# alvinliu0/HumanGaussian

Measured on AMD Instinct MI355X. Metric: rasterize fwd+bwd Gaussians/sec @1024^2, 100k pts, higher is better.
Workload: dtype f32

## Files before the change

humangaussian_amd/csrc/api.hip:

```cpp
#include "hgs_common.h"
#include <stdio.h>
#include <stdlib.h>
#include <string.h>
#include <algorithm>
#include <atomic>
#include <mutex>

#ifdef HGS_TIMELINE
__device__ unsigned long long hgs_tl[HGS_TL_KERNELS][HGS_TL_SLOTS][4];
#endif
#include "preprocess.hip"
#include "binning.hip"
#include "render_fwd.hip"
#include "knn.hip"
#include "mesh.hip"
#include "fields.hip"
#include "bookkeeping.hip"
#include "optim.hip"
#include "lbs.hip"
#include "pose.hip"
#include "step_images.hip"
#include "surface.hip"

extern "C" __global__ void hgs_k_render_bwd(View, Layout, const hgs_status*, const SortRec*, const float*,
// ... 4 lines not shown

namespace {

#ifdef HGS_KNOBS
inline int hgs_knob(const char* name, int dflt) { const char* e = getenv(name); return (e && atoi(e) > 0) ? atoi(e) : dflt; }
#else
inline int hgs_knob(const char*, int dflt) { return dflt; }
#endif

#define HGS_CHUNK_ROWS_MIN_VIEWS 3
#ifndef HGS_PRE_BWD_VPAR_MIN_VIEWS
#define HGS_PRE_BWD_VPAR_MIN_VIEWS 2
#endif
constexpr size_t ALIGN = 256;
struct Carver {
  size_t off = 0;
  size_t take(size_t bytes) { const size_t o = off; off = hgs_align_up(off + bytes, ALIGN); return o; }
};
struct ScanShape { unsigned blocks; size_t bsum_bytes; };
inline ScanShape scan_shape(size_t n, size_t elem) {
  const size_t nb = (n + HGS_SCAN_BLOCK - 1) / HGS_SCAN_BLOCK;
  return {(unsigned)nb, (nb + 1) * elem};
}
constexpr size_t HGS_LDS_BINS_MAX = 16384;
#define HGS_BIN_WGS_PER_VIEW_MAX 512
#define HGS_BIN_WGS_TOTAL_MAX 1024
constexpr int HGS_MAX_BIN_WGS_PER_VIEW = HGS_BIN_WGS_PER_VIEW_MAX;
constexpr int HGS_BIN_WGS_TOTAL = HGS_BIN_WGS_TOTAL_MAX;

struct GeomCarve {
  size_t geom, tile_n, tile_start, tile_order, tile_rec, cell_info, items_part, fwd_cells,
      hist, tile_gbase, tile_count, chunk_sums, chunk_base, ctr, status, total;
};

inline int grid_dim(int pixels) { return (pixels + HGS_TILE - 1) / HGS_TILE; }

inline void bin_shape(int B, int P, int& nblk, int& cpw, int& nwg) {
  nblk = (P + HGS_BLOCK - 1) / HGS_BLOCK;
  int want = HGS_BIN_WGS_TOTAL / (B > 0 ? B : 1);
  if (want > HGS_MAX_BIN_WGS_PER_VIEW) want = HGS_MAX_BIN_WGS_PER_VIEW;
  if (want < 1) want = 1;
  cpw = (nblk + want - 1) / want;
  if (cpw < 1) cpw = 1;
  nwg = (nblk + cpw - 1) / cpw;
}

GeomCarve carve_geom(int B, int P, int H, int W) {
  const size_t T = (size_t)grid_dim(W) * grid_dim(H);
  const size_t TT = T * (size_t)B;
  int nblk, cpw, nwg;
  bin_shape(B, P, nblk, cpw, nwg);
  const bool lds = T <= HGS_LDS_BINS_MAX;
  GeomCarve c;
  Carver cv;
  c.geom = cv.take((size_t)B * P * sizeof(GeomRec));
  c.tile_n = cv.take(TT * 4);
  c.tile_start = cv.take(TT * 4);
  c.tile_order = cv.take(TT * 4);
  c.tile_rec = cv.take(TT * 16);
  c.cell_info = cv.take(TT * 16 * sizeof(CellInfo));
  const size_t dcap = hgs_die_cells((int)TT);
  c.items_part = cv.take(HGS_NXCD * 2 * dcap * sizeof(uint4));
  c.fwd_cells = cv.take((size_t)HGS_NXCD * HGS_NFC * dcap * 4);
  c.hist = cv.take(lds ? (size_t)B * nwg * T * 4 : 0);
  c.tile_gbase = cv.take(lds ? (size_t)HGS_ROW_GROUPS * TT * 4 : 0);
  c.tile_count = cv.take(lds ? 0 : TT * 4);
  c.chunk_sums = cv.take((size_t)B * nblk * 4);
  c.chunk_base = cv.take((size_t)B * nblk * 4);
  c.ctr = cv.take(sizeof(Counters));
  c.status = cv.take(sizeof(hgs_status));
  c.total = cv.off;
  return c;
}

// ... 25 lines not shown
  L.tile_start = reinterpret_cast<uint32_t*>(gp + g.tile_start);
  L.tile_order = reinterpret_cast<uint32_t*>(gp + g.tile_order);
  L.tile_rec = reinterpret_cast<uint4*>(gp + g.tile_rec);
  L.cell_info = reinterpret_cast<CellInfo*>(gp + g.cell_info);
  L.items_part = reinterpret_cast<uint4*>(gp + g.items_part);
  L.fwd_cells = reinterpret_cast<uint32_t*>(gp + g.fwd_cells);
  L.hist = reinterpret_cast<uint32_t*>(gp + g.hist);
  L.tile_gbase = reinterpret_cast<uint32_t*>(gp + g.tile_gbase);
  L.tile_count = reinterpret_cast<uint32_t*>(gp + g.tile_count);
  L.chunk_sums = reinterpret_cast<uint32_t*>(gp + g.chunk_sums);
  L.chunk_base = reinterpret_cast<uint32_t*>(gp + g.chunk_base);
  L.ctr = reinterpret_cast<Counters*>(gp + g.ctr);
  L.keys = bp ? reinterpret_cast<unsigned long long*>(bp + b.keys) : nullptr;
  L.recs = bp ? reinterpret_cast<SortRec*>(bp + b.recs) : nullptr;
  L.cell_list = bp ? reinterpret_cast<uint2*>(bp + b.cell_list) : nullptr;
  L.entpair = bp ? reinterpret_cast<uint2*>(bp + b.entpair) : nullptr;
  L.cstate = bp ? reinterpret_cast<float*>(bp + b.cstate) : nullptr;
  L.items_full = bp ? reinterpret_cast<uint4*>(bp + b.items_full) : nullptr;
  L.full_cap = (uint32_t)((size_t)(cap > 0 ? cap : 0) * HGS_PAIRS_PER_ENTRY / HGS_SEGLEN + 1);
  L.n_contrib = static_cast<uint32_t*>(img);
  return L;
}

View make_view(const hgs_settings* s, int B, int P, int M, int64_t cap, int max_tile_hint = 0, int act = 0) {
  View v;
  v.act = act;
  v.pairchunks = B >= HGS_CHUNK_ROWS_MIN_VIEWS ? 1 : 0;
  for (int b = 0; b < HGS_MAX_VIEWS; ++b) {
    const hgs_settings& sb = s[b < B ? b : 0];
    Cam& c = v.cam[b];
    c.viewmatrix = sb.viewmatrix;
    c.projmatrix = sb.projmatrix;
    c.campos = sb.campos;
    c.bg = sb.bg;
    c.tanfovx = sb.tanfovx;
    c.tanfovy = sb.tanfovy;
    c.focal_x = (float)sb.image_width / (2.0f * sb.tanfovx);
    c.focal_y = (float)sb.image_height / (2.0f * sb.tanfovy);
  }
  v.scale_modifier = s->scale_modifier;
  v.W = s->image_width;
  v.H = s->image_height;
  v.grid_x = grid_dim(v.W);
  v.grid_y = grid_dim(v.H);
  v.T = v.grid_x * v.grid_y;
  v.B = B;
  v.TT = B * v.T;
  v.P = P;
  v.M = M;
  v.D = s->sh_degree;
  v.lds_bins = (size_t)v.T <= HGS_LDS_BINS_MAX ? 1 : 0;
  bin_shape(B, P, v.nblk, v.cpw, v.nwg);
  if (!v.lds_bins) { v.cpw = 1; v.nwg = v.nblk; }
  v.entry_capacity = (uint32_t)(cap < 0 ? 0 : (cap > 0xffffffffll ? 0xffffffffll : cap));
  v.max_tile_hint = max_tile_hint;
  return v;
}

inline int hip_rc(hipError_t e) { return e == hipSuccess ? HGS_OK : -(1000 + (int)e); }

inline hipError_t box_init(void* hdr, size_t hdr_bytes, uint32_t* bmin, hipStream_t stream) {
  const hipError_t e = hipMemsetAsync(hdr, 0, hdr_bytes, stream);
  return e != hipSuccess ? e : hipMemsetAsync(bmin, 0xff, 3 * sizeof(uint32_t), stream);
}

#define HGS_LAUNCH_CHECK()                       \
  do {                                           \
    hipError_t e__ = hipGetLastError();          \
    if (e__ != hipSuccess) return hip_rc(e__);   \
  } while (0)

#define HGS_STAGE(k)                                                              \
  do {                                                                            \
    if (stage_events && stage_events[k]) {                                        \
      hipError_t e__ = hipEventRecord(static_cast<hipEvent_t>(stage_events[k]), stream); \
// ... 240 lines not shown

int hgs_forward_batch_act(const hgs_settings* s, int32_t B, int32_t P, int32_t M, const float* means3D,
                          const float* shs, const float* colors_precomp, const float* opacities,
                          const float* scales, const float* rotations, const float* cov3D_precomp,
                          float* out_color, float* out_depth, float* out_alpha, int32_t* radii,
                          void* geom, void* bin, int64_t entry_capacity, void* img,
                          int32_t store_bwd_state, int32_t max_tile_entries_hint, hgs_status* status_host,
                          int32_t status_host_mapped, void* status_event, void* const* stage_events,
                          int32_t activation_flags, void* stream_) {
  return hgs_forward_batch_act_leaf(s, B, P, M, means3D, shs, colors_precomp, opacities, scales, rotations, cov3D_precomp,
                                    out_color, out_depth, out_alpha, radii, geom, bin, entry_capacity, img, store_bwd_state,
                                    max_tile_entries_hint, status_host, status_host_mapped, status_event, stage_events,
                                    activation_flags, nullptr, stream_);
}

int hgs_forward_batch_act_leaf(const hgs_settings* s, int32_t B, int32_t P, int32_t M, const float* means3D,
                               const float* shs, const float* colors_precomp, const float* opacities,
                               const float* scales, const float* rotations, const float* cov3D_precomp,
                               float* out_color, float* out_depth, float* out_alpha, int32_t* radii,
                               void* geom, void* bin, int64_t entry_capacity, void* img,
                               int32_t store_bwd_state, int32_t max_tile_entries_hint, hgs_status* status_host,
                               int32_t status_host_mapped, void* status_event, void* const* stage_events,
                               int32_t activation_flags, float* means2D_leaf, void* stream_) {
  if (activation_flags & ~(7 | HGS_GRAD_SCALE_TRUE_DERIVATIVE | HGS_ANTIALIAS)) return HGS_EINVAL;
  if (!batch_ok(s, B) || P < 0 || !out_color || !out_depth || !out_alpha || !geom || !img ||
      entry_capacity < 0)
    return HGS_EINVAL;
  if (P > 0) {
    if (!means3D || !opacities || !radii) return HGS_EINVAL;
    if ((shs != nullptr) == (colors_precomp != nullptr)) return HGS_ESHAPE;
    const bool has_sr = scales != nullptr && rotations != nullptr;
    if ((scales != nullptr) != (rotations != nullptr)) return HGS_ESHAPE;
    if (has_sr == (cov3D_precomp != nullptr)) return HGS_ESHAPE;
    if (shs && M < (s->sh_degree + 1) * (s->sh_degree + 1)) return HGS_ESHAPE;
    if (entry_capacity > 0 && !bin) return HGS_EINVAL;
    if ((int64_t)B * P >= (1ll << 31) || P >= (1 << 28)) return HGS_EINVAL;
  }
  if (entry_capacity > HGS_MAX_ENTRY_CAPACITY) return HGS_EINVAL;
  hipStream_t stream = static_cast<hipStream_t>(stream_);
  DeviceState* const ds = device_state(stream);
  const int ncu = cu_count(ds);
  const bool aa = (activation_flags & HGS_ANTIALIAS) != 0;
  const View v = make_view(s, B, P, M, entry_capacity, max_tile_entries_hint > 0 ? max_tile_entries_hint : 0,
                           activation_flags & 7);
  const Layout L = make_layout(geom, bin, img, B, P, v.H, v.W, entry_capacity);
  hgs_status* status_dev =
      reinterpret_cast<hgs_status*>(static_cast<char*>(geom) + carve_geom(B, P, v.H, v.W).status);

  HGS_STAGE(0);
  hipError_t e = hipSuccess;
  if (v.nblk == 0) {
    e = hipMemsetAsync(L.ctr, 0, sizeof(Counters), stream);
    if (e != hipSuccess) return hip_rc(e);
  }
  const size_t lds_bytes = (size_t)v.T * 4;
  if (!v.lds_bins) {
    e = hipMemsetAsync(L.tile_count, 0, (size_t)v.TT * 4, stream);
    if (e != hipSuccess) return hip_rc(e);
  }
  if (v.nblk > 0) {
    if (v.lds_bins)
      hipLaunchKernelGGL(aa ? hgs_k_preprocess_fwd_aa : hgs_k_preprocess_fwd, dim3(v.B * v.nwg), dim3(HGS_BLOCK), lds_bytes,
                         stream, v, L, means3D, shs, colors_precomp, opacities, scales, rotations,
                         cov3D_precomp, radii, means2D_leaf);
    else
      hipLaunchKernelGGL(aa ? hgs_k_preprocess_fwd_ga_aa : hgs_k_preprocess_fwd_ga, dim3(v.B * v.nblk), dim3(HGS_BLOCK), 0,
                         stream, v, L, means3D, shs, colors_precomp, opacities, scales, rotations,
                         cov3D_precomp, radii, means2D_leaf);
    HGS_LAUNCH_CHECK();
  }
  HGS_STAGE(1);
  const unsigned bpv = (unsigned)((v.T + HGS_TILES_PER_WG - 1) / HGS_TILES_PER_WG);
  hipLaunchKernelGGL(hgs_k_tiles, dim3(bpv * (unsigned)v.B), dim3(64 * HGS_ROW_GROUPS), 0, stream, v, L);
  HGS_LAUNCH_CHECK();
  HGS_STAGE(2);
  const unsigned order_wgs = (unsigned)((v.TT + HGS_BLOCK - 1) / HGS_BLOCK);
  hgs_status* status_mapped = status_host_mapped ? status_host : nullptr;
  const unsigned nbin = entry_capacity > 0 ? (unsigned)(v.B * (v.lds_bins ? v.nwg : v.nblk)) : 0u;
  if (v.lds_bins && nbin)
    hipLaunchKernelGGL(hgs_k_fill, dim3(nbin + order_wgs), dim3(HGS_BLOCK), lds_bytes, stream, v, L, status_dev,
                       status_mapped, (int)nbin);
  else
    hipLaunchKernelGGL(hgs_k_fill_ga, dim3(nbin + order_wgs), dim3(HGS_BLOCK), 0, stream, v, L, status_dev,
                       status_mapped, (int)nbin);
  HGS_LAUNCH_CHECK();
  if (status_host && !status_host_mapped) {
    e = hipMemcpyAsync(status_host, status_dev, sizeof(hgs_status), hipMemcpyDeviceToHost, stream);
    if (e != hipSuccess) return hip_rc(e);
  }
  if (status_event) {
    e = hipEventRecord(static_cast<hipEvent_t>(status_event), stream);
    if (e != hipSuccess) return hip_rc(e);
  }
  if (entry_capacity > 0) {
    HGS_STAGE(3);
    auto class_grid = [&](int64_t lo) {
      const int64_t g = entry_capacity / lo + 1;
      return (unsigned)(g < v.TT ? g : v.TT);
    };
    const int hint = v.max_tile_hint;
    const bool need_huge = hint <= 0 || hint > 16384, need_large = hint <= 0 || hint > HGS_SORT_LDS_MAX;
    const bool expect_long = hint <= 0 || hint > HGS_SORT_LDS_MAX + HGS_SORT_LDS_MAX / 2 + 64;
// ... 909 lines not shown
```

humangaussian_amd/csrc/binning.hip:

```cpp
#include "hgs_common.h"

extern "C" __global__ void __launch_bounds__(64 * HGS_ROW_GROUPS)
hgs_k_tiles(View v, Layout L) {
  __shared__ uint32_t gt[HGS_ROW_GROUPS][HGS_TILES_PER_WG];
  __shared__ uint32_t start_s[HGS_TILES_PER_WG];
  __shared__ uint32_t cls_s[HGS_NCLS];
  const int tid = threadIdx.x, tl = tid & 63;
  const int rg = __builtin_amdgcn_readfirstlane(tid >> 6);
  const int bpv = (v.T + HGS_TILES_PER_WG - 1) / HGS_TILES_PER_WG;
  const int b = (int)blockIdx.x / bpv;
  const int t = ((int)blockIdx.x % bpv) * HGS_TILES_PER_WG + tl;
  const bool valid = t < v.T;
  const size_t g = (size_t)b * v.T + t;
  if (tid < HGS_NCLS) cls_s[tid] = 0;
  uint32_t run = 0;
  if (v.lds_bins) {
    const int rpg = (v.nwg + HGS_ROW_GROUPS - 1) / HGS_ROW_GROUPS;
    const int r0 = rg * rpg, r1 = min(v.nwg, r0 + rpg);
    if (valid) {
      uint32_t* col = L.hist + (size_t)b * v.nwg * v.T + t;
      constexpr int BR = 16;
      for (int r = r0; r < r1; r += BR) {
        uint32_t c[BR];
#pragma unroll
// ... 77 lines not shown
      const uint32_t* sw = reinterpret_cast<const uint32_t*>(&st);
      for (int k = 0; k < 7; ++k) hs[k] = sw[k];
      __threadfence_system();
      hs[7] = 1u;
      __threadfence_system();
    }
  }
  if (tid >= 128 && tid < 192) {
    const int nchunk = v.B * v.nblk;
    const int per_wg = (nchunk + nblks - 1) / nblks;
    const int c_begin = blk * per_wg, c_end = min(nchunk, c_begin + per_wg);
    for (int c0 = c_begin; c0 < c_end; c0 += 64) {
      const int c = c0 + lane;
      const uint32_t sum = (c < c_end) ? L.chunk_sums[c] : 0u;
      const uint32_t inc = hgs_wave_incl_scan(sum);
      uint32_t base = 0;
      if (lane == 63 && inc) base = atomicAdd(&L.ctr->entry_alloc, inc);
      base = (uint32_t)__builtin_amdgcn_readlane((int)base, 63);
      if (c < c_end) L.chunk_base[c] = base + inc - sum;
    }
  }
  __syncthreads();
  const int g = blk * HGS_BLOCK + tid;
  const bool valid = g < v.TT;
  const uint32_t n = valid ? L.tile_n[g] : 0u;
  const int c = (valid && n) ? 32 - __clz(n) : 0;
  int leader_of = 0;
  uint32_t rank = 0, cnt = 0;
  unsigned long long todo = __ballot(valid);
  while (todo) {
    const int leader = (int)__builtin_ctzll(todo);
    const int cl = __builtin_amdgcn_readlane(c, leader);
    const unsigned long long same = __ballot(valid && c == cl);
    if (valid && c == cl) {
      leader_of = leader;
      rank = __builtin_amdgcn_mbcnt_hi((uint32_t)(same >> 32), __builtin_amdgcn_mbcnt_lo((uint32_t)same, 0u));
      cnt = (uint32_t)__popcll(same);
    }
    todo &= ~same;
  }
  uint32_t base = 0;
  if (valid && lane == leader_of) base = atomicAdd(&L.ctr->cls_cur[c].v, cnt);
  base = (uint32_t)__shfl((int)base, leader_of, 64);
  const uint32_t pos = cls_base[c] + base + rank;
  if (!valid) return;
  L.tile_order[pos] = (uint32_t)g;
  L.tile_rec[pos] = make_uint4((uint32_t)g, n, L.tile_start[g], 0u);
}

extern "C" __global__ void __launch_bounds__(HGS_BLOCK)
hgs_k_fill(View v, Layout L, hgs_status* __restrict__ status, hgs_status* __restrict__ status_host, int nbin) {
  extern __shared__ __attribute__((aligned(16))) uint32_t lds_cur[];
  if ((int)blockIdx.x >= nbin) {
    place_tiles(v, L, (int)blockIdx.x - nbin, (int)gridDim.x - nbin, status, status_host);
    return;
  }
  if (overflow_from_counters(v, L)) return;
  const int b = (int)blockIdx.x / v.nwg, lw = (int)blockIdx.x % v.nwg;
  const uint32_t* __restrict__ base_row = L.hist + (size_t)blockIdx.x * v.T;
  const int rpg = (v.nwg + HGS_ROW_GROUPS - 1) / HGS_ROW_GROUPS;
  const uint32_t* __restrict__ grp_row = L.tile_gbase + (size_t)(lw / rpg) * v.TT + (size_t)b * v.T;
  for (int t = threadIdx.x; t < v.T; t += HGS_BLOCK) lds_cur[t] = grp_row[t] + base_row[t];
  __syncthreads();
  const GeomRec* __restrict__ geom = L.geom + (size_t)b * v.P;
  for (int c = 0; c < v.cpw; ++c) {
    const int chunk = lw * v.cpw + c;
    if (chunk >= v.nblk) break;
    const int i = chunk * HGS_BLOCK + threadIdx.x;
    if (i >= v.P) continue;
    const uint4 q2 = reinterpret_cast<const uint4*>(&geom[i])[2];
    const uint32_t depth_bits = q2.y, lo = q2.z, hi = q2.w;
    const int minx = lo & 0xffffu, miny = lo >> 16, maxx = hi & 0xffffu, maxy = hi >> 16;
    const unsigned long long key_hi = (unsigned long long)depth_bits << 32;
    for (int ty = miny; ty < maxy; ++ty)
      for (int tx = minx; tx < maxx; ++tx) {
        const uint32_t slot = atomicAdd(&lds_cur[ty * v.grid_x + tx], 1u);
        L.keys[slot] = key_hi | (uint32_t)i;
      }
  }
}

extern "C" __global__ void __launch_bounds__(HGS_BLOCK)
hgs_k_fill_ga(View v, Layout L, hgs_status* __restrict__ status, hgs_status* __restrict__ status_host, int nbin) {
  if ((int)blockIdx.x >= nbin) {
    place_tiles(v, L, (int)blockIdx.x - nbin, (int)gridDim.x - nbin, status, status_host);
    return;
  }
  if (overflow_from_counters(v, L)) return;
  const int b = (int)blockIdx.x / v.nblk, chunk = (int)blockIdx.x % v.nblk;
  const int i = chunk * HGS_BLOCK + threadIdx.x;
  if (i >= v.P) return;
  const uint4 q2 = reinterpret_cast<const uint4*>(&L.geom[(size_t)b * v.P + i])[2];
  const uint32_t depth_bits = q2.y, lo = q2.z, hi = q2.w;
  const int minx = lo & 0xffffu, miny = lo >> 16, maxx = hi & 0xffffu, maxy = hi >> 16;
  const unsigned long long key_hi = (unsigned long long)depth_bits << 32;
  for (int ty = miny; ty < maxy; ++ty)
    for (int tx = minx; tx < maxx; ++tx) {
      const size_t g = (size_t)b * v.T + ty * v.grid_x + tx;
      const uint32_t slot = L.tile_start[g] + atomicAdd(&L.tile_count[g], 1u);
      L.keys[slot] = key_hi | (uint32_t)i;
    }
}
// ... 966 lines not shown
```

humangaussian_amd/csrc/hgs_common.h:

```cpp
#pragma once
#include <hip/hip_runtime.h>
#include <stdint.h>

#include "../../include/hgs_rast.h"
#include "cellmask.h"
#include "entryrec.h"

#define HGS_TILE 16
#define HGS_TILE_PIX 256
#define HGS_BLOCK 256
#define HGS_ROW_GROUPS 16
#define HGS_TILES_PER_WG 64
#define HGS_RB 16
#define HGS_ROW_F4 (HGS_RB * HGS_REC_F4 + 1)
#define HGS_BWD_BLOCK_WAVES 12
#define HGS_SEGLEN 128
#define HGS_NEAR_Z 0.2f
#define HGS_ALPHA_MIN (1.0f / 255.0f)
#define HGS_ALPHA_MAX 0.99f
#define HGS_T_EPS 0.0001f
#define HGS_CSTATE_FLOATS (6 * 16)
#define HGS_ROW_FLOATS 12
#define HGS_GROW_F4 (HGS_ROW_FLOATS / 4)
#define HGS_PROW_FLOATS 10
// ... 69 lines not shown
  float* cstate;
  uint32_t full_cap;
  uint4* items_full;
  uint32_t* n_contrib;
};

__host__ __device__ __forceinline__ size_t hgs_die_cells(int TT) { return (size_t)16 * (size_t)((TT + HGS_NXCD - 1) / HGS_NXCD); }

struct Cam {
  const float* viewmatrix;
  const float* projmatrix;
  const float* campos;
  const float* bg;
  float tanfovx, tanfovy, focal_x, focal_y;
};

struct View {
  Cam cam[HGS_MAX_VIEWS];
  float scale_modifier;
  int32_t W, H, grid_x, grid_y, T;
  int32_t B, TT;
  int32_t P, M, D, nblk;
  int32_t cpw, nwg, lds_bins;
  uint32_t entry_capacity;
  int32_t max_tile_hint;
  int32_t act;
  int32_t pairchunks;
};

static inline size_t hgs_align_up(size_t v, size_t a) { return (v + a - 1) / a * a; }

__device__ __forceinline__ int hgs_cell_of(int w, int j) { return (((w >> 1) << 1) + (j >> 1)) * 4 + ((w & 1) << 1) + (j & 1); }
#define HGS_FWD_THREADS 256

__device__ __forceinline__ bool hgs_eval_alpha(float dx, float dy, float qa, float qb,
                                               float qc, float op, float& G, float& alpha,
                                               float& m2, float& m3) {
  m2 = __builtin_fmaf(qa, dx, qb * dy);
  m3 = qc * dy;
  const float p2 = __builtin_fmaf(dx, m2, m3 * dy);
  G = __builtin_amdgcn_exp2f(p2);
  const float og = op * G;
  alpha = fminf(HGS_ALPHA_MAX, og);
  return (p2 <= 0.0f) && (og >= HGS_ALPHA_MIN);
}

// ... 86 lines not shown
```

humangaussian_amd/csrc/preprocess.hip:

```cpp
#include "hgs_common.h"

namespace {

__device__ __constant__ const float SH_C0 = 0.28209479177387814f;
__device__ __constant__ const float SH_C1 = 0.4886025119029199f;
__device__ __constant__ const float SH_C2[5] = {1.0925484305920792f, -1.0925484305920792f,
                                                0.31539156525252005f, -1.0925484305920792f,
                                                0.5462742152960396f};
__device__ __constant__ const float SH_C3[7] = {-0.5900435899266435f, 2.890611442640554f,
                                                -0.4570457994644658f, 0.3731763325901154f,
                                                -0.4570457994644658f, 1.445305721320277f,
                                                -0.5900435899266435f};

struct Cov3 { float c0, c1, c2, c3, c4, c5; };

struct RotScale {
  float R00, R01, R02, R10, R11, R12, R20, R21, R22;
  float sx, sy, sz;
};

__device__ __forceinline__ float act_opacity(float raw, int act) {
  return (act & HGS_ACT_OPACITY_SIGMOID) ? 1.0f / (1.0f + expf(-raw)) : raw;
}
__device__ __forceinline__ void act_scale(const float* __restrict__ scales, int i, int act, float& s0, float& s1, float& s2) {
// ... 277 lines not shown
      col[ch] = col[ch] + 0.5f;
      if (col[ch] < 0.0f) { cl |= (1u << ch); col[ch] = 0.0f; }
    }
    rec.r = col[0]; rec.g = col[1]; rec.b = col[2];
    rec.clamped = cl;
  }
  return (uint32_t)tight_area;
}

__device__ __forceinline__ void store_geom(GeomRec* dstp, const GeomRec& rec) {
  uint4* dst = reinterpret_cast<uint4*>(dstp);
  const uint4* src = reinterpret_cast<const uint4*>(&rec);
  dst[0] = src[0]; dst[1] = src[1]; dst[2] = src[2]; dst[3] = src[3];
}

}

__device__ __forceinline__ uint32_t chunk_prefix(uint32_t tt, uint32_t* wtot, uint32_t* chunk_sum) {
  uint32_t total;
  const uint32_t ex = hgs_block_excl_scan<HGS_BLOCK>(tt, wtot, total);
  if (threadIdx.x == 0) *chunk_sum = total;
  return ex;
}

__device__ __forceinline__ void zero_counters(const Layout& L) {
  if (blockIdx.x == 0)
    for (uint32_t i = threadIdx.x; i < sizeof(Counters) / 4; i += blockDim.x) reinterpret_cast<uint32_t*>(L.ctr)[i] = 0u;
}

template <bool AA>
__device__ __forceinline__ void preprocess_fwd_body(
    const View& v, const Layout& L, const float* __restrict__ means3D, const float* __restrict__ shs,
    const float* __restrict__ colors_precomp, const float* __restrict__ opacities, const float* __restrict__ scales,
    const float* __restrict__ rotations, const float* __restrict__ cov3D_precomp, int32_t* __restrict__ radii,
    float* __restrict__ zero_leaf) {
  extern __shared__ __attribute__((aligned(16))) uint32_t lds_hist[];
  __shared__ uint32_t wtot[HGS_BLOCK / 64];
  zero_counters(L);
  const int b = (int)blockIdx.x / v.nwg, lw = (int)blockIdx.x % v.nwg;
  const Cam cam = v.cam[b];
  for (int t = threadIdx.x; t < v.T; t += HGS_BLOCK) lds_hist[t] = 0u;
  __syncthreads();
  const int gxm = v.grid_x;
  for (int c = 0; c < v.cpw; ++c) {
    const int chunk = lw * v.cpw + c;
    if (chunk >= v.nblk) break;
    const int i = chunk * HGS_BLOCK + threadIdx.x;
    uint32_t tt = 0;
    if (i < v.P) {
      GeomRec rec;
      tt = preprocess_one<AA>(v, cam, i, means3D, shs, colors_precomp, opacities, scales, rotations,
                              cov3D_precomp, rec);
      radii[(size_t)b * v.P + i] = rec.radius;
      if (zero_leaf) {
        float* z = zero_leaf + ((size_t)b * v.P + i) * 3;
        z[0] = 0.0f; z[1] = 0.0f; z[2] = 0.0f;
      }
      store_geom(&L.geom[(size_t)b * v.P + i], rec);
      if (tt) {
        const int minx = rec.rect_lo & 0xffffu, miny = rec.rect_lo >> 16;
        const int maxx = rec.rect_hi & 0xffffu, maxy = rec.rect_hi >> 16;
        for (int ty = miny; ty < maxy; ++ty)
          for (int tx = minx; tx < maxx; ++tx) atomicAdd(&lds_hist[ty * gxm + tx], 1u);
      }
    }
    const uint32_t off = chunk_prefix(tt, wtot, &L.chunk_sums[(size_t)b * v.nblk + chunk]);
    if (i < v.P && tt) L.geom[(size_t)b * v.P + i].offset = off;
  }
  __syncthreads();
  uint32_t* row = L.hist + (size_t)blockIdx.x * v.T;
  for (int t = threadIdx.x; t < v.T; t += HGS_BLOCK) row[t] = lds_hist[t];
}

template <bool AA>
__device__ __forceinline__ void preprocess_fwd_ga_body(
    const View& v, const Layout& L, const float* __restrict__ means3D, const float* __restrict__ shs,
    const float* __restrict__ colors_precomp, const float* __restrict__ opacities, const float* __restrict__ scales,
    const float* __restrict__ rotations, const float* __restrict__ cov3D_precomp, int32_t* __restrict__ radii,
    float* __restrict__ zero_leaf) {
  __shared__ uint32_t wtot[HGS_BLOCK / 64];
  zero_counters(L);
  const int b = (int)blockIdx.x / v.nblk, chunk = (int)blockIdx.x % v.nblk;
  const Cam cam = v.cam[b];
  const int i = chunk * HGS_BLOCK + threadIdx.x;
  uint32_t tt = 0;
  if (i < v.P) {
    GeomRec rec;
    tt = preprocess_one<AA>(v, cam, i, means3D, shs, colors_precomp, opacities, scales, rotations,
                            cov3D_precomp, rec);
    radii[(size_t)b * v.P + i] = rec.radius;
    if (zero_leaf) {
      float* z = zero_leaf + ((size_t)b * v.P + i) * 3;
      z[0] = 0.0f; z[1] = 0.0f; z[2] = 0.0f;
    }
    store_geom(&L.geom[(size_t)b * v.P + i], rec);
    if (tt) {
      const int minx = rec.rect_lo & 0xffffu, miny = rec.rect_lo >> 16;
      const int maxx = rec.rect_hi & 0xffffu, maxy = rec.rect_hi >> 16;
      uint32_t* cnt = L.tile_count + (size_t)b * v.T;
      for (int ty = miny; ty < maxy; ++ty)
        for (int tx = minx; tx < maxx; ++tx) atomicAdd(&cnt[ty * v.grid_x + tx], 1u);
    }
  }
  const uint32_t off = chunk_prefix(tt, wtot, &L.chunk_sums[blockIdx.x]);
  if (i < v.P && tt) L.geom[(size_t)b * v.P + i].offset = off;
}

#define HGS_PRE_FWD_KERNEL(NAME, BODY, AA)                                                                       \
  extern "C" __global__ void __launch_bounds__(HGS_BLOCK) NAME(                                                  \
      View v, Layout L, const float* __restrict__ means3D, const float* __restrict__ shs,                        \
      const float* __restrict__ colors_precomp, const float* __restrict__ opacities,                             \
      const float* __restrict__ scales, const float* __restrict__ rotations,                                     \
      const float* __restrict__ cov3D_precomp, int32_t* __restrict__ radii, float* __restrict__ zero_leaf) {     \
    BODY<AA>(v, L, means3D, shs, colors_precomp, opacities, scales, rotations, cov3D_precomp, radii, zero_leaf);   \
  }
HGS_PRE_FWD_KERNEL(hgs_k_preprocess_fwd, preprocess_fwd_body, false)
HGS_PRE_FWD_KERNEL(hgs_k_preprocess_fwd_ga, preprocess_fwd_ga_body, false)
HGS_PRE_FWD_KERNEL(hgs_k_preprocess_fwd_aa, preprocess_fwd_body, true)
HGS_PRE_FWD_KERNEL(hgs_k_preprocess_fwd_ga_aa, preprocess_fwd_ga_body, true)

namespace {

template <int DEG, int MODE, int AA>
__device__ __forceinline__ void preprocess_bwd_body(
    const View& v, const Layout& L, const hgs_status* __restrict__ status,
    const float* __restrict__ grad_rows, const float* __restrict__ means3D,
    const float* __restrict__ shs, const float* __restrict__ colors_precomp,
    const float* __restrict__ opacities_raw,
    const float* __restrict__ scales, const float* __restrict__ rotations,
    const float* __restrict__ cov3D_precomp, float* __restrict__ dL_dmeans3D,
    float* __restrict__ dL_dmeans2D, float* __restrict__ dL_dshs, float* __restrict__ dL_dcolors,
    float* __restrict__ dL_dopac, float* __restrict__ dL_dscales, float* __restrict__ dL_drots,
    float* __restrict__ dL_dcov3D, float* __restrict__ pack, int pack_F) {
  constexpr int NC = (DEG + 1) * (DEG + 1);
  constexpr bool SINGLE = MODE != 0;
  constexpr bool VPAR = MODE == 2;
  constexpr int NV = 23 + 3 * NC;
  extern __shared__ float red[];
  int i = blockIdx.x * HGS_BLOCK + threadIdx.x, bview = 0, il = threadIdx.x;
  if (VPAR) {
    il = (int)threadIdx.x & 63;
    bview = __builtin_amdgcn_readfirstlane((int)threadIdx.x >> 6);
// ... 520 lines not shown
```

humangaussian_amd/csrc/torch_binding.cpp:

```cpp
#include <torch/extension.h>
#include <c10/hip/HIPFunctions.h>
#include <c10/hip/HIPStream.h>
#include <hip/hip_runtime_api.h>

#include <algorithm>
#include <atomic>
#include <chrono>
#include <thread>
#include <map>
#include <tuple>
#include <mutex>
#include <utility>
#include <stdexcept>
#include <string>
#include <vector>

#include "../../include/hgs_rast.h"

namespace {

using torch::Tensor;
using torch::autograd::AutogradContext;
using torch::autograd::variable_list;

// ... 244 lines not shown
      const int slot = st.ring_pos;
      st.ring_pos = (st.ring_pos + 1) % RING;
      st.ring_issued += 1;
      plan->slot = &st.ring[slot];
      plan->slot_issue = st.ring_issued;
      volatile uint32_t* ready = &st.ring[slot].reserved[2];
      *ready = 0u;
      std::atomic_thread_fence(std::memory_order_seq_cst);
      const auto th1 = std::chrono::steady_clock::now();
      if (attempt == 0) st.host_ns[0] += std::chrono::duration_cast<std::chrono::nanoseconds>(th1 - th0).count();
      const int rc = hgs_forward_batch_act_leaf(plan->settings.s.data(), (int32_t)B, (int32_t)P, M, fptr(m3), fptr(sh_), fptr(cp_),
                                                fptr(op_), fptr(sc_), fptr(ro_), fptr(cv_), fptr_mut(color), fptr_mut(depth),
                                                fptr_mut(alpha), P > 0 ? radii.data_ptr<int32_t>() : nullptr, plan->geom,
                                                plan->bin, cap, plan->img, want_grad ? 1 : 0, hint, &st.ring[slot], 1,
                                                nullptr, g_stage_fwd.empty() ? nullptr : g_stage_fwd.data(),
                                                (int32_t)act, leaf_ptr, stream);
      check_rc(rc, "hgs_forward_batch");
      const auto th2 = std::chrono::steady_clock::now();
      st.host_ns[1] += std::chrono::duration_cast<std::chrono::nanoseconds>(th2 - th1).count();
      if (debug) hip_ok(hipStreamSynchronize(stream), "device error in the rasterizer forward (debug=True)");
      if (attempt == 0 && want_grad) {
        plan->B = (int32_t)B; plan->P = (int32_t)P; plan->M = M;
        plan->batched = batched;
        plan->act = (int32_t)act;
        plan->has_sh = has_sh; plan->has_cp = has_cp; plan->has_sr = has_sc; plan->has_cv = has_cv;
        plan->opac_sizes = opacities.sizes().vec();
        variable_list saved = {m3, op_, radii, color, depth, alpha};
        for (const Tensor* t : {&sh_, &cp_, &sc_, &ro_, &cv_})
          if (t->defined()) saved.push_back(*t);
        ctx->save_for_backward(saved);
        plan->alloc_grads(plan->pre_grads, dev);
        plan->pre_stream = (void*)stream;
      }
      const auto tw = std::chrono::steady_clock::now();
      st.host_ns[2] += std::chrono::duration_cast<std::chrono::nanoseconds>(tw - th2).count();
      for (uint64_t spins = 0; *ready == 0u; ++spins) {
        if ((spins & 0x3ff) == 0x3ff) {
          if (std::chrono::steady_clock::now() - tw > std::chrono::seconds(2)) {
            hip_ok(hipStreamSynchronize(stream), "rasterizer forward");
            if (*ready == 0u) throw std::runtime_error("libhgs_rast: the forward finished without publishing its status");
            break;
          }
          std::this_thread::yield();
        }
      }
      std::atomic_thread_fence(std::memory_order_seq_cst);
      const int64_t waited = std::chrono::duration_cast<std::chrono::nanoseconds>(std::chrono::steady_clock::now() - tw).count();
// ... 1135 lines not shown
```

humangaussian_amd/rasterizer.py:

```python
from __future__ import annotations

from typing import NamedTuple, Optional

import torch
from torch import nn

from . import _lib


class GaussianRasterizationSettings(NamedTuple):
    image_height: int
    image_width: int
    tanfovx: float
    tanfovy: float
    bg: torch.Tensor
    scale_modifier: float
    viewmatrix: torch.Tensor
    projmatrix: torch.Tensor
    sh_degree: int
    campos: torch.Tensor
    prefiltered: bool
    debug: bool


# ... 23 lines not shown

def rasterize_gaussians(means3D, means2D, sh, colors_precomp, opacities, scales, rotations,
                        cov3Ds_precomp, raster_settings, zero_means2D: bool = False,
                        antialiasing: Optional[bool] = None):
    want_grad = torch.is_grad_enabled() and (
        means3D.requires_grad or means2D.requires_grad or opacities.requires_grad
        or (sh is not None and sh.requires_grad)
        or (colors_precomp is not None and colors_precomp.requires_grad)
        or (scales is not None and scales.requires_grad)
        or (rotations is not None and rotations.requires_grad)
        or (cov3Ds_precomp is not None and cov3Ds_precomp.requires_grad))
    rs = raster_settings
    aa = _settings_antialiasing(rs) if antialiasing is None else bool(antialiasing)
    color, radii, depth, alpha = _lib.load_binding().rasterize(
        means3D, means2D, sh, colors_precomp, opacities, scales, rotations, cov3Ds_precomp,
        rs.bg, rs.viewmatrix, rs.projmatrix, rs.campos, int(rs.image_height), int(rs.image_width),
        float(rs.tanfovx), float(rs.tanfovy), float(rs.scale_modifier), int(rs.sh_degree),
        bool(rs.prefiltered), bool(rs.debug), want_grad, bool(zero_means2D), ANTIALIAS if aa else 0)
    return color, radii, depth, alpha


ACT_OPACITY_SIGMOID, ACT_SCALE_EXP, ACT_ROTATION_NORMALIZE = 1, 2, 4
ANTIALIAS = 16
ZERO_MEANS2D = 1 << 16
GRAD_SCALE_TRUE_DERIVATIVE = 8


def rasterize_gaussians_batch(means3D, means2D, sh, colors_precomp, opacities, scales, rotations,
                              cov3Ds_precomp, raster_settings_list, activation_flags: int = 0,
                              antialiasing: Optional[bool] = None):
    rsl = list(raster_settings_list)
    if not rsl:
        raise ValueError("rasterize_gaussians_batch needs at least one view")
    r0 = rsl[0]
    for rs in rsl[1:]:
        if (int(rs.image_height), int(rs.image_width), int(rs.sh_degree), float(rs.scale_modifier)) != \
                (int(r0.image_height), int(r0.image_width), int(r0.sh_degree), float(r0.scale_modifier)):
            raise ValueError("all views of a batch must share image size, sh_degree and scale_modifier")
        if _settings_antialiasing(rs) != _settings_antialiasing(r0):
            raise ValueError("all views of a batch must agree in antialiasing")
    if antialiasing is None:
        antialiasing = bool(int(activation_flags) & ANTIALIAS) or _settings_antialiasing(r0)
    activation_flags = (int(activation_flags) & ~ANTIALIAS) | (ANTIALIAS if antialiasing else 0)
    B = len(rsl)
    dev = means3D.device
    if B == 1:
# ... 71 lines not shown
```

include/hgs_rast.h:

```cpp
#ifndef HGS_RAST_H
#define HGS_RAST_H

#include <stddef.h>
#include <stdint.h>

#ifdef __cplusplus
extern "C" {
#endif

#define HGS_MAX_VIEWS 16
#define HGS_MAX_ENTRY_CAPACITY (1ll << 27)

#define HGS_OK 0
#define HGS_EINVAL (-1)
#define HGS_ESHAPE (-2)

typedef struct hgs_settings {
  int32_t image_height;
  int32_t image_width;
  float tanfovx;
  float tanfovy;
  const float* bg;
  float scale_modifier;
  const float* viewmatrix;
// ... 43 lines not shown
                      int32_t store_bwd_state, int32_t max_tile_entries_hint,
                      hgs_status* status_host, int32_t status_host_mapped, void* status_event,
                      void* const* stage_events, void* stream);

int hgs_backward_batch(const hgs_settings* views, int32_t B, int32_t P, int32_t M,
                       const float* means3D, const float* shs, const float* colors_precomp,
                       const float* opacities, const float* scales, const float* rotations,
                       const float* cov3D_precomp, const int32_t* radii,
                       const float* out_color, const float* out_depth, const float* out_alpha,
                       const float* dL_dout_color, const float* dL_dout_depth,
                       const float* dL_dout_alpha,
                       const void* geom, const void* bin, const void* img,
                       const hgs_status* status, int64_t entry_capacity, void* bwd_scratch,
                       float* dL_dmeans3D, float* dL_dmeans2D, float* dL_dshs,
                       float* dL_dcolors_precomp, float* dL_dopacities, float* dL_dscales,
                       float* dL_drotations, float* dL_dcov3D_precomp,
                       void* const* stage_events, void* stream);

#define HGS_ACT_OPACITY_SIGMOID 1
#define HGS_ACT_SCALE_EXP 2
#define HGS_ACT_ROTATION_NORMALIZE 4
#define HGS_GRAD_SCALE_TRUE_DERIVATIVE 8
#define HGS_ANTIALIAS 16
int hgs_forward_batch_act(const hgs_settings* views, int32_t B, int32_t P, int32_t M,
                          const float* means3D, const float* shs, const float* colors_precomp,
                          const float* opacities, const float* scales, const float* rotations,
                          const float* cov3D_precomp,
                          float* out_color, float* out_depth, float* out_alpha, int32_t* radii,
                          void* geom, void* bin, int64_t entry_capacity, void* img,
                          int32_t store_bwd_state, int32_t max_tile_entries_hint,
                          hgs_status* status_host, int32_t status_host_mapped, void* status_event,
                          void* const* stage_events, int32_t activation_flags, void* stream);
int hgs_forward_batch_act_leaf(const hgs_settings* views, int32_t B, int32_t P, int32_t M,
                               const float* means3D, const float* shs, const float* colors_precomp,
                               const float* opacities, const float* scales, const float* rotations,
                               const float* cov3D_precomp,
                               float* out_color, float* out_depth, float* out_alpha, int32_t* radii,
                               void* geom, void* bin, int64_t entry_capacity, void* img,
                               int32_t store_bwd_state, int32_t max_tile_entries_hint,
                               hgs_status* status_host, int32_t status_host_mapped, void* status_event,
                               void* const* stage_events, int32_t activation_flags, float* means2D_leaf, void* stream);
int hgs_backward_batch_act(const hgs_settings* views, int32_t B, int32_t P, int32_t M,
                           const float* means3D, const float* shs, const float* colors_precomp,
                           const float* opacities, const float* scales, const float* rotations,
                           const float* cov3D_precomp, const int32_t* radii,
                           const float* out_color, const float* out_depth, const float* out_alpha,
// ... 268 lines not shown
```

Before: 658.4 million.

## Add wide 2-chunk workgroups for single-view preprocess and binning fill

For single-view batches whose chunk count exceeds the CU count, preprocess and fill now launch workgroups of twice the block size, each processing two point chunks at once. This halves the number of per-workgroup tile histogram rows that must be zeroed, written, scanned and read back in fill. It also keeps per-chunk prefix sums correct through a new wave-grouped scan. The cost is fewer, larger workgroups and a per-workgroup LDS histogram shared by more threads, which can increase atomic contention. New flags let callers force narrow or wide mode.

```diff
diff --git a/humangaussian_amd/csrc/api.hip b/humangaussian_amd/csrc/api.hip
--- a/humangaussian_amd/csrc/api.hip
+++ b/humangaussian_amd/csrc/api.hip
@@ -50,6 +50,7 @@
   const size_t nb = (n + HGS_SCAN_BLOCK - 1) / HGS_SCAN_BLOCK;
   return {(unsigned)nb, (nb + 1) * elem};
 }
+#define HGS_BIN_BITS (HGS_BIN_NARROW | HGS_BIN_WIDE)
 constexpr size_t HGS_LDS_BINS_MAX = 16384;
 #define HGS_BIN_WGS_PER_VIEW_MAX 512
 #define HGS_BIN_WGS_TOTAL_MAX 1024
@@ -63,21 +64,29 @@
 
 inline int grid_dim(int pixels) { return (pixels + HGS_TILE - 1) / HGS_TILE; }
 
-inline void bin_shape(int B, int P, int& nblk, int& cpw, int& nwg) {
+inline void bin_shape(int B, int P, bool wide, int& nblk, int& cpw, int& nwg) {
   nblk = (P + HGS_BLOCK - 1) / HGS_BLOCK;
   int want = HGS_BIN_WGS_TOTAL / (B > 0 ? B : 1);
   if (want > HGS_MAX_BIN_WGS_PER_VIEW) want = HGS_MAX_BIN_WGS_PER_VIEW;
   if (want < 1) want = 1;
   cpw = (nblk + want - 1) / want;
   if (cpw < 1) cpw = 1;
+  if (wide) cpw = (cpw + 1) & ~1;
   nwg = (nblk + cpw - 1) / cpw;
+}
+
+inline bool bin_wide(int flags, int B, int P, int ncu) {
+  if (B != 1 || (flags & HGS_BIN_NARROW)) return false;
+  if (flags & HGS_BIN_WIDE) return true;
+  const int nblk = (P + HGS_BLOCK - 1) / HGS_BLOCK;
+  return nblk > ncu && nblk <= HGS_MAX_BIN_WGS_PER_VIEW;
 }
 
 GeomCarve carve_geom(int B, int P, int H, int W) {
   const size_t T = (size_t)grid_dim(W) * grid_dim(H);
   const size_t TT = T * (size_t)B;
   int nblk, cpw, nwg;
-  bin_shape(B, P, nblk, cpw, nwg);
+  bin_shape(B, P, false, nblk, cpw, nwg);
   const bool lds = T <= HGS_LDS_BINS_MAX;
   GeomCarve c;
   Carver cv;
@@ -149,7 +158,7 @@
   return L;
 }
 
-View make_view(const hgs_settings* s, int B, int P, int M, int64_t cap, int max_tile_hint = 0, int act = 0) {
+View make_view(const hgs_settings* s, int B, int P, int M, int64_t cap, int max_tile_hint = 0, int act = 0, bool wide = false) {
   View v;
   v.act = act;
   v.pairchunks = B >= HGS_CHUNK_ROWS_MIN_VIEWS ? 1 : 0;
@@ -177,7 +186,8 @@
   v.M = M;
   v.D = s->sh_degree;
   v.lds_bins = (size_t)v.T <= HGS_LDS_BINS_MAX ? 1 : 0;
-  bin_shape(B, P, v.nblk, v.cpw, v.nwg);
+  v.wide = (wide && v.lds_bins && B == 1) ? 1 : 0;
+  bin_shape(B, P, v.wide != 0, v.nblk, v.cpw, v.nwg);
   if (!v.lds_bins) { v.cpw = 1; v.nwg = v.nblk; }
   v.entry_capacity = (uint32_t)(cap < 0 ? 0 : (cap > 0xffffffffll ? 0xffffffffll : cap));
   v.max_tile_hint = max_tile_hint;
@@ -464,7 +474,8 @@
                                int32_t store_bwd_state, int32_t max_tile_entries_hint, hgs_status* status_host,
                                int32_t status_host_mapped, void* status_event, void* const* stage_events,
                                int32_t activation_flags, float* means2D_leaf, void* stream_) {
-  if (activation_flags & ~(7 | HGS_GRAD_SCALE_TRUE_DERIVATIVE | HGS_ANTIALIAS)) return HGS_EINVAL;
+  if (activation_flags & ~(7 | HGS_GRAD_SCALE_TRUE_DERIVATIVE | HGS_ANTIALIAS | HGS_BIN_BITS)) return HGS_EINVAL;
+  if ((activation_flags & HGS_BIN_BITS) == HGS_BIN_BITS) return HGS_EINVAL;
   if (!batch_ok(s, B) || P < 0 || !out_color || !out_depth || !out_alpha || !geom || !img ||
       entry_capacity < 0)
     return HGS_EINVAL;
@@ -484,7 +495,7 @@
   const int ncu = cu_count(ds);
   const bool aa = (activation_flags & HGS_ANTIALIAS) != 0;
   const View v = make_view(s, B, P, M, entry_capacity, max_tile_entries_hint > 0 ? max_tile_entries_hint : 0,
-                           activation_flags & 7);
+                           activation_flags & 7, bin_wide(activation_flags, B, P, ncu));
   const Layout L = make_layout(geom, bin, img, B, P, v.H, v.W, entry_capacity);
   hgs_status* status_dev =
       reinterpret_cast<hgs_status*>(static_cast<char*>(geom) + carve_geom(B, P, v.H, v.W).status);
@@ -501,7 +512,11 @@
     if (e != hipSuccess) return hip_rc(e);
   }
   if (v.nblk > 0) {
-    if (v.lds_bins)
+    if (v.wide)
+      hipLaunchKernelGGL(aa ? hgs_k_preprocess_fwd_w_aa : hgs_k_preprocess_fwd_w, dim3(v.nwg), dim3(2 * HGS_BLOCK), lds_bytes,
+                         stream, v, L, means3D, shs, colors_precomp, opacities, scales, rotations,
+                         cov3D_precomp, radii, means2D_leaf);
+    else if (v.lds_bins)
       hipLaunchKernelGGL(aa ? hgs_k_preprocess_fwd_aa : hgs_k_preprocess_fwd, dim3(v.B * v.nwg), dim3(HGS_BLOCK), lds_bytes,
                          stream, v, L, means3D, shs, colors_precomp, opacities, scales, rotations,
                          cov3D_precomp, radii, means2D_leaf);
@@ -519,7 +534,10 @@
   const unsigned order_wgs = (unsigned)((v.TT + HGS_BLOCK - 1) / HGS_BLOCK);
   hgs_status* status_mapped = status_host_mapped ? status_host : nullptr;
   const unsigned nbin = entry_capacity > 0 ? (unsigned)(v.B * (v.lds_bins ? v.nwg : v.nblk)) : 0u;
-  if (v.lds_bins && nbin)
+  if (v.wide && nbin)
+    hipLaunchKernelGGL(hgs_k_fill_w, dim3(nbin + order_wgs), dim3(2 * HGS_BLOCK), lds_bytes, stream, v, L, status_dev,
+                       status_mapped, (int)nbin);
+  else if (v.lds_bins && nbin)
     hipLaunchKernelGGL(hgs_k_fill, dim3(nbin + order_wgs), dim3(HGS_BLOCK), lds_bytes, stream, v, L, status_dev,
                        status_mapped, (int)nbin);
   else
diff --git a/humangaussian_amd/csrc/binning.hip b/humangaussian_amd/csrc/binning.hip
--- a/humangaussian_amd/csrc/binning.hip
+++ b/humangaussian_amd/csrc/binning.hip
@@ -123,7 +123,7 @@
   }
   __syncthreads();
   const int g = blk * HGS_BLOCK + tid;
-  const bool valid = g < v.TT;
+  const bool valid = g < v.TT && tid < HGS_BLOCK;
   const uint32_t n = valid ? L.tile_n[g] : 0u;
   const int c = (valid && n) ? 32 - __clz(n) : 0;
   int leader_of = 0;
@@ -149,8 +149,9 @@
   L.tile_rec[pos] = make_uint4((uint32_t)g, n, L.tile_start[g], 0u);
 }
 
-extern "C" __global__ void __launch_bounds__(HGS_BLOCK)
-hgs_k_fill(View v, Layout L, hgs_status* __restrict__ status, hgs_status* __restrict__ status_host, int nbin) {
+template <int NCH>
+__device__ __forceinline__ void fill_body(const View& v, const Layout& L, hgs_status* __restrict__ status,
+                                          hgs_status* __restrict__ status_host, int nbin) {
   extern __shared__ __attribute__((aligned(16))) uint32_t lds_cur[];
   if ((int)blockIdx.x >= nbin) {
     place_tiles(v, L, (int)blockIdx.x - nbin, (int)gridDim.x - nbin, status, status_host);
@@ -161,13 +162,14 @@
   const uint32_t* __restrict__ base_row = L.hist + (size_t)blockIdx.x * v.T;
   const int rpg = (v.nwg + HGS_ROW_GROUPS - 1) / HGS_ROW_GROUPS;
   const uint32_t* __restrict__ grp_row = L.tile_gbase + (size_t)(lw / rpg) * v.TT + (size_t)b * v.T;
-  for (int t = threadIdx.x; t < v.T; t += HGS_BLOCK) lds_cur[t] = grp_row[t] + base_row[t];
+  for (int t = threadIdx.x; t < v.T; t += NCH * HGS_BLOCK) lds_cur[t] = grp_row[t] + base_row[t];
   __syncthreads();
   const GeomRec* __restrict__ geom = L.geom + (size_t)b * v.P;
-  for (int c = 0; c < v.cpw; ++c) {
+  const int half = NCH == 1 ? 0 : (int)threadIdx.x / HGS_BLOCK, tl = (int)threadIdx.x % HGS_BLOCK;
+  for (int c = half; c < v.cpw; c += NCH) {
     const int chunk = lw * v.cpw + c;
     if (chunk >= v.nblk) break;
-    const int i = chunk * HGS_BLOCK + threadIdx.x;
+    const int i = chunk * HGS_BLOCK + tl;
     if (i >= v.P) continue;
     const uint4 q2 = reinterpret_cast<const uint4*>(&geom[i])[2];
     const uint32_t depth_bits = q2.y, lo = q2.z, hi = q2.w;
@@ -179,6 +181,14 @@
         L.keys[slot] = key_hi | (uint32_t)i;
       }
   }
+}
+extern "C" __global__ void __launch_bounds__(HGS_BLOCK)
+hgs_k_fill(View v, Layout L, hgs_status* __restrict__ status, hgs_status* __restrict__ status_host, int nbin) {
+  fill_body<1>(v, L, status, status_host, nbin);
+}
+extern "C" __global__ void __launch_bounds__(2 * HGS_BLOCK)
+hgs_k_fill_w(View v, Layout L, hgs_status* __restrict__ status, hgs_status* __restrict__ status_host, int nbin) {
+  fill_body<2>(v, L, status, status_host, nbin);
 }
 
 extern "C" __global__ void __launch_bounds__(HGS_BLOCK)
diff --git a/humangaussian_amd/csrc/hgs_common.h b/humangaussian_amd/csrc/hgs_common.h
--- a/humangaussian_amd/csrc/hgs_common.h
+++ b/humangaussian_amd/csrc/hgs_common.h
@@ -115,6 +115,7 @@
   int32_t B, TT;
   int32_t P, M, D, nblk;
   int32_t cpw, nwg, lds_bins;
+  int32_t wide;
   uint32_t entry_capacity;
   int32_t max_tile_hint;
   int32_t act;
diff --git a/humangaussian_amd/csrc/preprocess.hip b/humangaussian_amd/csrc/preprocess.hip
--- a/humangaussian_amd/csrc/preprocess.hip
+++ b/humangaussian_amd/csrc/preprocess.hip
@@ -323,32 +323,50 @@
   if (threadIdx.x == 0) *chunk_sum = total;
   return ex;
 }
+__device__ __forceinline__ uint32_t chunk_prefix_wide(uint32_t tt, uint32_t* wtot, uint32_t* chunk_sum) {
+  const int lane = threadIdx.x & 63, w = threadIdx.x >> 6, w0 = w & ~3;
+  const uint32_t incl = hgs_wave_incl_scan(tt);
+  __syncthreads();
+  if (lane == 63) wtot[w] = incl;
+  __syncthreads();
+  uint32_t base = 0, tot = 0;
+#pragma unroll
+  for (int k = 0; k < HGS_BLOCK / 64; ++k) {
+    const uint32_t t = wtot[w0 + k];
+    if (w0 + k < w) base += t;
+    tot += t;
+  }
+  if ((threadIdx.x & (HGS_BLOCK - 1)) == 0 && chunk_sum) *chunk_sum = tot;
+  return base + incl - tt;
+}
 
 __device__ __forceinline__ void zero_counters(const Layout& L) {
   if (blockIdx.x == 0)
     for (uint32_t i = threadIdx.x; i < sizeof(Counters) / 4; i += blockDim.x) reinterpret_cast<uint32_t*>(L.ctr)[i] = 0u;
 }
 
-template <bool AA>
+template <bool AA, int NCH>
 __device__ __forceinline__ void preprocess_fwd_body(
     const View& v, const Layout& L, const float* __restrict__ means3D, const float* __restrict__ shs,
     const float* __restrict__ colors_precomp, const float* __restrict__ opacities, const float* __restrict__ scales,
     const float* __restrict__ rotations, const float* __restrict__ cov3D_precomp, int32_t* __restrict__ radii,
     float* __restrict__ zero_leaf) {
   extern __shared__ __attribute__((aligned(16))) uint32_t lds_hist[];
-  __shared__ uint32_t wtot[HGS_BLOCK / 64];
+  __shared__ uint32_t wtot[NCH * HGS_BLOCK / 64];
   zero_counters(L);
   const int b = (int)blockIdx.x / v.nwg, lw = (int)blockIdx.x % v.nwg;
   const Cam cam = v.cam[b];
-  for (int t = threadIdx.x; t < v.T; t += HGS_BLOCK) lds_hist[t] = 0u;
+  for (int t = threadIdx.x; t < v.T; t += NCH * HGS_BLOCK) lds_hist[t] = 0u;
   __syncthreads();
   const int gxm = v.grid_x;
-  for (int c = 0; c < v.cpw; ++c) {
-    const int chunk = lw * v.cpw + c;
-    if (chunk >= v.nblk) break;
-    const int i = chunk * HGS_BLOCK + threadIdx.x;
+  const int half = NCH == 1 ? 0 : (int)threadIdx.x / HGS_BLOCK, tl = (int)threadIdx.x % HGS_BLOCK;
+  for (int c = 0; c < v.cpw; c += NCH) {
+    if (lw * v.cpw + c >= v.nblk) break;
+    const int chunk = lw * v.cpw + c + half;
+    const bool has = NCH == 1 || chunk < v.nblk;
+    const int i = chunk * HGS_BLOCK + tl;
     uint32_t tt = 0;
-    if (i < v.P) {
+    if (has && i < v.P) {
       GeomRec rec;
       tt = preprocess_one<AA>(v, cam, i, means3D, shs, colors_precomp, opacities, scales, rotations,
                               cov3D_precomp, rec);
@@ -365,15 +383,16 @@
           for (int tx = minx; tx < maxx; ++tx) atomicAdd(&lds_hist[ty * gxm + tx], 1u);
       }
     }
-    const uint32_t off = chunk_prefix(tt, wtot, &L.chunk_sums[(size_t)b * v.nblk + chunk]);
-    if (i < v.P && tt) L.geom[(size_t)b * v.P + i].offset = off;
+    uint32_t* const chunk_sum = &L.chunk_sums[(size_t)b * v.nblk + chunk];
+    const uint32_t off = NCH == 1 ? chunk_prefix(tt, wtot, chunk_sum) : chunk_prefix_wide(tt, wtot, has ? chunk_sum : nullptr);
+    if (has && i < v.P && tt) L.geom[(size_t)b * v.P + i].offset = off;
   }
   __syncthreads();
   uint32_t* row = L.hist + (size_t)blockIdx.x * v.T;
-  for (int t = threadIdx.x; t < v.T; t += HGS_BLOCK) row[t] = lds_hist[t];
-}
-
-template <bool AA>
+  for (int t = threadIdx.x; t < v.T; t += NCH * HGS_BLOCK) row[t] = lds_hist[t];
+}
+
+template <bool AA, int NCH>
 __device__ __forceinline__ void preprocess_fwd_ga_body(
     const View& v, const Layout& L, const float* __restrict__ means3D, const float* __restrict__ shs,
     const float* __restrict__ colors_precomp, const float* __restrict__ opacities, const float* __restrict__ scales,
@@ -407,18 +426,20 @@
   if (i < v.P && tt) L.geom[(size_t)b * v.P + i].offset = off;
 }
 
-#define HGS_PRE_FWD_KERNEL(NAME, BODY, AA)                                                                       \
-  extern "C" __global__ void __launch_bounds__(HGS_BLOCK) NAME(                                                  \
+#define HGS_PRE_FWD_KERNEL(NAME, BODY, AA, NCH)                                                                  \
+  extern "C" __global__ void __launch_bounds__(NCH * HGS_BLOCK) NAME(                                            \
       View v, Layout L, const float* __restrict__ means3D, const float* __restrict__ shs,                        \
       const float* __restrict__ colors_precomp, const float* __restrict__ opacities,                             \
       const float* __restrict__ scales, const float* __restrict__ rotations,                                     \
       const float* __restrict__ cov3D_precomp, int32_t* __restrict__ radii, float* __restrict__ zero_leaf) {     \
-    BODY<AA>(v, L, means3D, shs, colors_precomp, opacities, scales, rotations, cov3D_precomp, radii, zero_leaf);   \
-  }
-HGS_PRE_FWD_KERNEL(hgs_k_preprocess_fwd, preprocess_fwd_body, false)
-HGS_PRE_FWD_KERNEL(hgs_k_preprocess_fwd_ga, preprocess_fwd_ga_body, false)
-HGS_PRE_FWD_KERNEL(hgs_k_preprocess_fwd_aa, preprocess_fwd_body, true)
-HGS_PRE_FWD_KERNEL(hgs_k_preprocess_fwd_ga_aa, preprocess_fwd_ga_body, true)
+    BODY<AA, NCH>(v, L, means3D, shs, colors_precomp, opacities, scales, rotations, cov3D_precomp, radii, zero_leaf); \
+  }
+HGS_PRE_FWD_KERNEL(hgs_k_preprocess_fwd, preprocess_fwd_body, false, 1)
+HGS_PRE_FWD_KERNEL(hgs_k_preprocess_fwd_ga, preprocess_fwd_ga_body, false, 1)
+HGS_PRE_FWD_KERNEL(hgs_k_preprocess_fwd_aa, preprocess_fwd_body, true, 1)
+HGS_PRE_FWD_KERNEL(hgs_k_preprocess_fwd_ga_aa, preprocess_fwd_ga_body, true, 1)
+HGS_PRE_FWD_KERNEL(hgs_k_preprocess_fwd_w, preprocess_fwd_body, false, 2)
+HGS_PRE_FWD_KERNEL(hgs_k_preprocess_fwd_w_aa, preprocess_fwd_body, true, 2)
 
 namespace {
 
diff --git a/humangaussian_amd/csrc/torch_binding.cpp b/humangaussian_amd/csrc/torch_binding.cpp
--- a/humangaussian_amd/csrc/torch_binding.cpp
+++ b/humangaussian_amd/csrc/torch_binding.cpp
@@ -290,7 +290,7 @@
       if (attempt == 0 && want_grad) {
         plan->B = (int32_t)B; plan->P = (int32_t)P; plan->M = M;
         plan->batched = batched;
-        plan->act = (int32_t)act;
+        plan->act = (int32_t)act & ~(HGS_BIN_NARROW | HGS_BIN_WIDE);
         plan->has_sh = has_sh; plan->has_cp = has_cp; plan->has_sr = has_sc; plan->has_cv = has_cv;
         plan->opac_sizes = opacities.sizes().vec();
         variable_list saved = {m3, op_, radii, color, depth, alpha};
diff --git a/humangaussian_amd/rasterizer.py b/humangaussian_amd/rasterizer.py
--- a/humangaussian_amd/rasterizer.py
+++ b/humangaussian_amd/rasterizer.py
@@ -69,6 +69,7 @@
 
 ACT_OPACITY_SIGMOID, ACT_SCALE_EXP, ACT_ROTATION_NORMALIZE = 1, 2, 4
 ANTIALIAS = 16
+BIN_NARROW, BIN_WIDE = 32, 64
 ZERO_MEANS2D = 1 << 16
 GRAD_SCALE_TRUE_DERIVATIVE = 8
 
diff --git a/include/hgs_rast.h b/include/hgs_rast.h
--- a/include/hgs_rast.h
+++ b/include/hgs_rast.h
@@ -89,6 +89,8 @@
 #define HGS_ACT_ROTATION_NORMALIZE 4
 #define HGS_GRAD_SCALE_TRUE_DERIVATIVE 8
 #define HGS_ANTIALIAS 16
+#define HGS_BIN_NARROW 32
+#define HGS_BIN_WIDE 64
 int hgs_forward_batch_act(const hgs_settings* views, int32_t B, int32_t P, int32_t M,
                           const float* means3D, const float* shs, const float* colors_precomp,
                           const float* opacities, const float* scales, const float* rotations,
```

New measurement: 653.9 million (median of 2 runs). No clear change (-0.7%).
